# SYSTRAN/faster-whisper

Measured on AMD Instinct MI355X. Metric: audio-sec/sec (RTF) large-v3 fp16 beam=5 batch=16, higher is better.
Workload: dtype f16

## Files before the change

faster_whisper_amd/_lib.py:

```python
import ctypes as C
import os

import numpy as np

_HERE = os.path.dirname(os.path.abspath(__file__))
LIB_PATH = os.environ.get("FWAMD_LIB") or os.path.join(_HERE, "libfwamd.so")

FW_OK = 0
FW_EINVAL = -1
FW_ENODEV = -2
FW_ENOMEM = -3
FW_ERUNTIME = -4
FW_ENOSPC = -5

COMPUTE_FLOAT16 = 0
COMPUTE_INT8_FLOAT16 = 1
FW_DT_F32 = 0
FW_DT_F16 = 1
FW_MAX_ALIGN_HEADS = 64
FW_MAX_ALTERNATIVES = 8


class FwConfig(C.Structure):
    _fields_ = [
        ("n_mels", C.c_int32), ("n_audio_ctx", C.c_int32), ("d_model", C.c_int32), ("n_heads", C.c_int32),
        ("n_enc_layers", C.c_int32), ("n_dec_layers", C.c_int32), ("n_vocab", C.c_int32),
        ("n_text_ctx", C.c_int32), ("is_multilingual", C.c_int32),
        ("tok_eot", C.c_int32), ("tok_sot", C.c_int32), ("tok_lang_begin", C.c_int32), ("n_langs", C.c_int32),
        ("tok_translate", C.c_int32), ("tok_transcribe", C.c_int32), ("tok_sot_lm", C.c_int32),
        ("tok_sot_prev", C.c_int32), ("tok_no_speech", C.c_int32), ("tok_no_timestamps", C.c_int32),
        ("tok_timestamp_begin", C.c_int32),
        ("n_suppress_begin", C.c_int32), ("suppress_begin", C.c_int32 * 8),
        ("n_align_heads", C.c_int32), ("align_heads", C.c_int32 * (2 * FW_MAX_ALIGN_HEADS)),
    ]


class FwWeight(C.Structure):
    _fields_ = [("name", C.c_char_p), ("data", C.c_void_p), ("dtype", C.c_int32), ("ndim", C.c_int32),
                ("dims", C.c_int64 * 4)]


class FwGenOpts(C.Structure):
    _fields_ = [
        ("beam_size", C.c_int32), ("patience", C.c_float), ("num_hypotheses", C.c_int32),
        ("length_penalty", C.c_float), ("repetition_penalty", C.c_float), ("no_repeat_ngram_size", C.c_int32),
        ("max_length", C.c_int32), ("return_scores", C.c_int32), ("return_no_speech_prob", C.c_int32),
        ("max_initial_timestamp_index", C.c_int32), ("suppress_blank", C.c_int32),
        ("suppress_tokens", C.POINTER(C.c_int32)), ("n_suppress_tokens", C.c_int32),
        ("sampling_topk", C.c_int32), ("sampling_temperature", C.c_float), ("seed", C.c_uint64),
        ("min_new_tokens", C.c_int32),
    ]


class FwVadWeights(C.Structure):
    _fields_ = [
        ("stft_basis", C.c_void_p), ("conv_w", C.c_void_p * 4), ("conv_b", C.c_void_p * 4),
        ("lstm_w", C.c_void_p), ("lstm_r", C.c_void_p), ("lstm_b", C.c_void_p), ("dec_w", C.c_void_p),
        ("dec_b", C.c_float),
    ]


SYMBOLS = [
    "fw_last_error", "fw_abi_version", "fw_device_count",
    "fw_model_create", "fw_model_free", "fw_model_info", "fw_model_blob", "fw_model_create_from_blob_dev",
    "fw_model_set_decode_batch", "fw_model_decode_batch", "fw_model_join_decoder", "fw_model_decode_stats",
    "fw_model_set_merge_wait", "fw_model_set_decode_lanes", "fw_model_run_capacity", "fw_dec_big_min_rows", "fw_dec_big_min_rows_of", "fw_test_knob",
    "fw_test_idle_lead_chunks", "fw_test_run_capacity", "fw_test_dec_linear_plan", "fw_test_self_attn_form",
    "fw_test_gemm_plan",
    "fw_pack_blob_size", "fw_pack_blob_copy", "fw_pack_blob_free",
    "fw_logmel", "fw_logmel_full",
    "fw_encode", "fw_encode_pcm", "fw_encode_pcm_dev", "fw_tensor_shape", "fw_tensor_to_host",
    "fw_tensor_from_host", "fw_tensor_free",
    "fw_generate", "fw_generate_lp", "fw_generate_alt", "fw_detect_language", "fw_align", "fw_score",
    "fw_prof_enable", "fw_prof_reset", "fw_prof_count", "fw_prof_name", "fw_prof_get", "fw_synchronize",
    "fw_dev_alloc", "fw_dev_free", "fw_dev_upload",
    "fw_test_gemm", "fw_test_layernorm", "fw_test_attention", "fw_test_dec_linear", "fw_test_dec_logits", "fw_test_logits_rules",
    "fw_test_dec_self_attn", "fw_test_dec_cross_attn", "fw_test_dec_cross_probs", "fw_test_dec_softmax_pick", "fw_bench_gemm", "fw_bench_dec_linear", "fw_bench_attention",
    "fw_bench_gemm_epi", "fw_bench_dec_linear_epi",
    "fw_test_gemm_ex", "fw_test_cross_kv_frag_index", "fw_test_quant_rows", "fw_test_layernorm_frag",
    "fw_test_dec_beam_update", "fw_test_dec_embed", "fw_test_align_post",
    "fw_test_logits_rules_lp", "fw_test_dec_beam_update_lp",
    "fw_test_logits_rules_alt", "fw_test_dec_beam_update_alt", "fw_test_alt_gather",
    "fw_test_logits_rules_smp_tab", "fw_test_logits_rules_ex", "fw_test_score_rows", "fw_test_graph_captures", "fw_test_blob_check",
    "fw_vad_create", "fw_vad_forward", "fw_vad_free", "fw_vad_forward_dev", "fw_vad_forward_audio_dev",
    "fw_vad_forward_audio_batch_dev",
    "fw_flac_info", "fw_flac_decode",
    "fw_resample_filter", "fw_resample_dev", "fw_bench_resample",
]

_lib = None


class FwError(RuntimeError):
    pass


def load():
    global _lib
    if _lib is not None:
        return _lib
    if not os.path.exists(LIB_PATH):
        raise FwError(
            f"{LIB_PATH} not found: build it with `python -c 'import __graft_entry__ as g; g.build()'` "
            "(hipcc --offload-arch=gfx950). faster_whisper_amd has no CPU fallback.")
    lib = C.CDLL(LIB_PATH)
    vp, i32, i64, f32p = C.c_void_p, C.c_int32, C.c_int64, C.POINTER(C.c_float)
    i32p, i64p = C.POINTER(C.c_int32), C.POINTER(C.c_int64)
    lib.fw_last_error.restype = C.c_char_p
    lib.fw_abi_version.restype = i32
    lib.fw_device_count.restype = i32
    lib.fw_model_create.argtypes = [C.POINTER(FwConfig), C.POINTER(FwWeight), i32, i32, i32, i32, i32, C.POINTER(vp)]
    lib.fw_model_free.argtypes = [vp]
    lib.fw_model_free.restype = None
    lib.fw_model_info.argtypes = [vp, C.POINTER(FwConfig), i32p, i32p, i32p, i32p]
    lib.fw_model_blob.argtypes = [vp, C.POINTER(vp), i64p]
    lib.fw_model_create_from_blob_dev.argtypes = [C.POINTER(FwConfig), vp, i64, i32, i32, i32, i32, C.POINTER(vp)]
    lib.fw_model_set_decode_batch.argtypes = [vp, i32]
    lib.fw_model_decode_batch.argtypes = [vp]
    lib.fw_model_decode_batch.restype = i32
    lib.fw_model_run_capacity.argtypes = [vp]
    lib.fw_model_run_capacity.restype = i32
    lib.fw_dec_big_min_rows.restype = i32
    if hasattr(lib, "fw_dec_big_min_rows_of"):
        lib.fw_dec_big_min_rows_of.restype = i32
        lib.fw_dec_big_min_rows_of.argtypes = [i32, i32]
    if hasattr(lib, "fw_flac_info"):
        lib.fw_flac_info.argtypes = [vp, i64, i32p, i32p, i32p, i64p]
        lib.fw_flac_decode.argtypes = [vp, i64, vp, i64, i64p, i32p]
    if hasattr(lib, "fw_test_knob"):
        lib.fw_test_knob.argtypes = [i32, i32]
    if hasattr(lib, "fw_test_idle_lead_chunks"):
        lib.fw_test_idle_lead_chunks.argtypes = [i64, i32, i32, i64, i32]
        lib.fw_test_idle_lead_chunks.restype = i64
    if hasattr(lib, "fw_test_run_capacity"):
        lib.fw_test_run_capacity.argtypes = [i32, i32, i32, i64, i32, i32, i32, i32, i32, i64p, i64p, i64p]
        lib.fw_test_run_capacity.restype = i32
    if hasattr(lib, "fw_test_dec_linear_plan"):
        lib.fw_test_dec_linear_plan.argtypes = [i32, i32, i32, i32, i32, i32, i32, i32p]
        lib.fw_test_self_attn_form.argtypes = [i32] * 8
        lib.fw_test_self_attn_form.restype = i32
    if hasattr(lib, "fw_test_gemm_plan"):
        lib.fw_test_gemm_plan.argtypes = [i32, i32, i32, i32, i64, i64, i64, i64, i64, i32, i32, i32, i32, i32, i32p]
    lib.fw_model_join_decoder.argtypes = [vp, vp]
    lib.fw_model_set_merge_wait.argtypes = [vp, i32, i32]
    lib.fw_model_set_decode_lanes.argtypes = [vp, i32]
    lib.fw_model_decode_stats.argtypes = [vp, i64p, i64p, i64p, i32p]
    lib.fw_pack_blob_size.argtypes = [C.POINTER(FwConfig), C.POINTER(FwWeight), i32, i32, i64p, C.POINTER(vp)]
    lib.fw_pack_blob_copy.argtypes = [vp, vp, i64]
    lib.fw_pack_blob_free.argtypes = [vp]
    lib.fw_pack_blob_free.restype = None
    lib.fw_logmel.argtypes = [vp, vp, i64p, i32, vp, i32p]
    lib.fw_logmel_full.argtypes = [vp, vp, i64, vp, i64]
    lib.fw_encode.argtypes = [vp, vp, i32, C.POINTER(vp)]
    lib.fw_encode_pcm.argtypes = [vp, vp, i64p, i32, C.POINTER(vp)]
    lib.fw_encode_pcm_dev.argtypes = [vp, vp, i64p, i32, C.POINTER(vp)]
    lib.fw_tensor_shape.argtypes = [vp, i32p, i32p, i32p]
    lib.fw_tensor_to_host.argtypes = [vp, vp, vp]
    lib.fw_tensor_from_host.argtypes = [vp, vp, i32, C.POINTER(vp)]
    lib.fw_tensor_free.argtypes = [vp]
    lib.fw_tensor_free.restype = None
    lib.fw_generate.argtypes = [vp, vp, i32p, i32p, i32, C.POINTER(FwGenOpts), i32p, i32p, f32p, f32p]
    if hasattr(lib, "fw_generate_lp"):
        lib.fw_generate_lp.argtypes = [vp, vp, i32p, i32p, i32, C.POINTER(FwGenOpts), i32p, i32p, f32p, f32p, f32p, f32p]
    if hasattr(lib, "fw_generate_alt"):
        f32 = C.c_float
        lib.fw_generate_alt.argtypes = [vp, vp, i32p, i32p, i32, C.POINTER(FwGenOpts), i32, i32p, i32p, f32p, f32p, f32p,
                                        f32p, i32p, f32p, i32p, f32p]
        lib.fw_test_logits_rules_alt.argtypes = [vp, vp, i32, vp, i32, vp, C.POINTER(FwGenOpts), i32, vp, vp, vp, vp, vp,
                                                 vp, vp, i32, vp, vp]
        lib.fw_test_dec_beam_update_alt.argtypes = [vp, i32, i32, i32, i32, i32, i32, i32, i32, f32, i32, vp, vp, vp, vp,
                                                    vp, vp, vp, i32, f32, vp, vp, vp, vp, vp, vp, vp, vp, vp, vp, vp, vp,
                                                    vp, vp, vp]
        lib.fw_test_alt_gather.argtypes = [vp, vp, vp, i32, i32, i32, i32, i32, vp, i32, vp, vp, vp, vp, i32, vp, vp]
    lib.fw_detect_language.argtypes = [vp, vp, i32, i32p, f32p]
    lib.fw_align.argtypes = [vp, vp, i32p, i32, i32p, i32p, i32p, i32, i32, i32, i32p, i32p, f32p]
    lib.fw_prof_enable.argtypes = [vp, i32]
    lib.fw_prof_enable.restype = None
    lib.fw_prof_reset.argtypes = [vp]
    lib.fw_prof_reset.restype = None
    lib.fw_prof_count.restype = i32
    lib.fw_prof_name.argtypes = [i32]
    lib.fw_prof_name.restype = C.c_char_p
    lib.fw_prof_get.argtypes = [vp, i32, C.POINTER(C.c_double), i64p, C.POINTER(C.c_double), C.POINTER(C.c_double)]
    lib.fw_synchronize.argtypes = [vp]
    lib.fw_dev_alloc.argtypes = [vp, i64, C.POINTER(vp)]
    lib.fw_dev_free.argtypes = [vp, vp]
    lib.fw_dev_upload.argtypes = [vp, vp, vp, i64]
    lib.fw_test_gemm.argtypes = [vp, vp, vp, vp, vp, i32, i32, i32, i32, i32, vp]
    lib.fw_test_dec_linear.argtypes = [vp, vp, vp, vp, vp, vp, vp, i32, i32, i32, i32, i32, vp, vp]
    lib.fw_test_dec_logits.argtypes = [vp, vp, i32, vp]
    lib.fw_test_logits_rules.argtypes = [vp, vp, i32, vp, i32, vp, C.POINTER(FwGenOpts), i32, vp, vp]
    if hasattr(lib, "fw_test_dec_self_attn"):
        lib.fw_test_dec_self_attn.argtypes = [vp, vp, vp, vp, vp, i32, i32, i32, i32, i32, i32, i32, i32, i32, i32, i32, vp]
        lib.fw_test_dec_cross_attn.argtypes = [vp, vp, vp, vp, i32, i32, i32, i32, i32, i32, vp, vp, i32, C.c_float, vp]
        lib.fw_test_dec_cross_probs.argtypes = [vp, vp, vp, i32, i32, i32, vp, i32, i32, i32, i32, vp]
# ... 78 lines not shown
```

faster_whisper_amd/csrc/gemm.hip:

```cpp
#include "common.h"
#include "kernels.h"
#include <atomic>
#include <type_traits>

#define GB_M 256
#define GB_N 256
#define GB_UNIT_BYTES (128 * 128)
#define GB_SLOT_BYTES (4 * GB_UNIT_BYTES)
#define GB_LDS_BYTES (8 * 64 * 272)

typedef int intx16 __attribute__((ext_vector_type(16)));

#ifndef GB_TL
#define GB_TL(slot)
#endif

#define GB_BARRIER()                      \
  do {                                    \
    asm volatile("" ::: "memory");         \
    __builtin_amdgcn_s_barrier();         \
    asm volatile("" ::: "memory");         \
  } while (0)

template <bool TRANS, bool I8, bool LAYERED = false>
// ... 406 lines not shown
            if (p.act == 1) v = gelu_erf(v);
            o[e] = (half_t)v;
          }
          half_t* dst = Cb + (size_t)n * p.ldc + m;
          if (m + 3 < p.M) {
            *reinterpret_cast<half4_t*>(dst) = o;
          } else {
#pragma unroll
            for (int e = 0; e < 4; ++e)
              if (m + e < p.M) dst[e] = o[e];
          }
        }
      }
  }
}

namespace fwk {

std::atomic<int> g_gemm_order{1};
std::atomic<int> g_gemm_vt_stage{1};

GemmPlan gemm_plan(const GemmParams& pin, int batch, bool trans) {
  GemmPlan pl{pin, -1, 0};
  GemmParams& p = pl.p;
  const bool i8 = p.a_scale != nullptr, layered = p.n_layers > 1;
  const int es = i8 ? 1 : 2;
  if (p.K <= 0 || (p.K * es) % 128 != 0) return pl;
  if (((p.lda * es) % 16) || ((p.ldw * es) % 16) || ((p.a_bstride * es) % 16)) return pl;
  if (!trans && ((p.N % 4) || (p.ldc % 4) || (p.c_bstride % 4))) return pl;
  if (i8 && !p.w_scale) return pl;
  if (layered && (i8 || p.res)) return pl;
  p.nMt = (p.M + GB_M - 1) / GB_M;
  p.nNt_layer = (p.N + GB_N - 1) / GB_N;
  p.nNt = p.nNt_layer * (layered ? p.n_layers : 1);
  p.n_mp = p.nMt * batch;
  p.blk_m = p.blk_n = 0;
  p.vt_stage = (trans && !i8 && p.head_rows == 0 && g_gemm_vt_stage.load(std::memory_order_relaxed) == 1 && p.ldc % 8 == 0 &&
                p.c_bstride % 8 == 0) ? 1 : 0;
  if (g_gemm_order.load(std::memory_order_relaxed) == 1 && p.nNt > 1 && p.n_mp > 1) {
    int bn = 1, best = 1 << 30;
    for (int c = 1; c <= p.nNt && c <= 16; ++c) {
      if (p.nNt % c) continue;
      const int cost = c + (32 + c - 1) / c;
      if (cost <= best) { best = cost; bn = c; }
    }
    p.blk_n = bn;
    p.blk_m = 32 / bn > 1 ? 32 / bn : 1;
  }
  pl.kernel = layered ? 4 + trans : 2 * i8 + trans;
  pl.grid = p.nMt * p.nNt * batch;
  return pl;
}

int launch_gemm(hipStream_t st, const GemmParams& pin, int batch, bool trans) {
  const GemmPlan pl = gemm_plan(pin, batch, trans);
  if (pl.kernel < 0) return -1;
  static void (*const kernels[6])(GemmParams) = {
      gemm_f16_kernel<false, false>, gemm_f16_kernel<true, false>,       gemm_f16_kernel<false, true>,
      gemm_f16_kernel<true, true>,   gemm_f16_kernel<false, false, true>, gemm_f16_kernel<true, false, true>};
  const int lds = GB_LDS_BYTES;
  static std::atomic<unsigned long long> attr_done{0};
  int dev = 0;
  (void)hipGetDevice(&dev);
  if (!((attr_done.load(std::memory_order_acquire) >> (dev & 63)) & 1ull)) {
    for (auto* k : kernels)
      (void)hipFuncSetAttribute(reinterpret_cast<const void*>(k), hipFuncAttributeMaxDynamicSharedMemorySize, lds);
    attr_done.fetch_or(1ull << (dev & 63), std::memory_order_release);
  }
  hipLaunchKernelGGL(kernels[pl.kernel], dim3(pl.grid), dim3(512), lds, st, pl.p);
  return 0;
}

}
```

faster_whisper_amd/csrc/hooks.hip:

```cpp
#include "engine.h"

#include <math.h>
#include <string.h>

#include <algorithm>

#include "dec_kernels.h"
#include "kernels.h"

using namespace fw;
using fwd::FIN_CAP;
using fwd::GenDev;

namespace {

struct HookBufs : DevBufs {
  template <typename T>
  int upload(T** dst, const T* src, size_t n) {
    int rc = alloc(dst, n);
    if (rc) return rc;
    FW_HIP(hipMemcpy(*dst, src, n * sizeof(T), hipMemcpyHostToDevice));
    return FW_OK;
  }
  int upload_f16(half_t** dst, const float* src, size_t n) {
// ... 182 lines not shown
        (rc = db.upload_f16(&d_x, x, (size_t)R * K)) || (bias && (rc = db.upload_f16(&d_bias, bias, N))) ||
        (rc = db.alloc(&d_xq, (size_t)R16 * K)) || (rc = db.alloc(&d_xs, (size_t)R16)) || (rc = db.zero(d_xq, (size_t)R16 * K, st)))
      return rc;
    fwk::launch_quant_rows(st, d_x, K, nullptr, nullptr, d_xq, d_xs, R, K, 1);
    if (fwd::launch_dec_gemm_frag_i8(st, d_xq, d_xs, d_wq, d_ws, d_bias, d_res, N, d_out, N, R, N, K, act) != 0) {
      set_error("int8 decoder linear: unsupported shape R=%d N=%d K=%d", R, N, K);
      return FW_ERUNTIME;
    }
    if ((rc = download_f16(st, out, d_out, (size_t)R * N))) return rc;
    memcpy(out_from_frag, out, (size_t)R * N * sizeof(float));
    return FW_OK;
  }
  std::vector<uint16_t> wf((size_t)N * K), xf((size_t)R16 * K, 0);
  std::vector<float> s1(N, 0.f), cf(N, 0.f);
  for (int n = 0; n < N; ++n) {
    double a1 = 0.0, ac = 0.0;
    for (int k = 0; k < K; ++k) {
      const float wv = h(W[(size_t)n * K + k]);
      const uint16_t wg = ln_g ? f32_to_f16_bits(wv * h(ln_g[k])) : f32_to_f16_bits(wv);
      wf[frag_pos(n, k, K, 32)] = wg;
      a1 += (double)f16_bits_to_f32(wg);
      if (ln_g) ac += (double)wv * (double)h(ln_b[k]);
    }
    if (bias) ac += (double)h(bias[n]);
    s1[n] = (float)a1;
    cf[n] = (float)ac;
  }
  for (int r = 0; r < R; ++r)
    for (int k = 0; k < K; ++k) xf[frag_pos(r, k, K, 32)] = f32_to_f16_bits(x[(size_t)r * K + k]);
  uint16_t *d_wf, *d_xf;
  half_t* d_of;
  float *d_s1 = nullptr, *d_cf = nullptr;
  if ((rc = db.upload(&d_wf, wf.data(), wf.size())) || (rc = db.upload(&d_xf, xf.data(), xf.size())) ||
      (rc = db.alloc(&d_of, (size_t)R16 * N)) || (rc = db.zero(d_of, (size_t)R16 * N * 2, st)))
    return rc;
  if (ln_g) {
    if ((rc = db.upload(&d_s1, s1.data(), (size_t)N)) || (rc = db.upload(&d_cf, cf.data(), (size_t)N))) return rc;
  } else if (bias) {
    if ((rc = db.upload_f16(&d_bias, bias, N))) return rc;
  }
  const fwd::DecLin lin{(const half_t*)d_xf, (const half_t*)d_wf, d_bias, d_s1, d_cf, d_res, N, d_out, N, d_of, R, N, K, act};
  if (fwd::launch_dec_linear(st, lin, form) != 0) {
    set_error("decoder linear: unsupported shape R=%d N=%d K=%d (form %d)", R, N, K, form);
    return FW_ERUNTIME;
  }
  if ((rc = download_f16(st, out, d_out, (size_t)R * N))) return rc;
  return download_f16_frag(st, out_from_frag, d_of, R, N);
}

int32_t fw_dec_big_min_rows(void) { return fwd::dec_big_min_rows(); }
int32_t fw_dec_big_min_rows_of(int32_t role, int32_t compute_type) { return fwd::dec_big_min_rows_of(role, compute_type); }

int32_t fw_test_knob(int32_t id, int32_t value) {
  FW_CHECK_ARG(id == 1 || id == 2 || id == 4 || id == 5 || id == 6 || id == 7, "unknown knob %d", id);
  if (id == 6) { set_cross_kv_layered(value); return FW_OK; }
  if (id == 7) { fwd::set_cross_attn_regs(value); return FW_OK; }
  if (id == 1) fwk::g_gemm_order.store(value);
  else if (id == 5) fwk::g_gemm_vt_stage.store(value);
  else if (id == 2) fwd::set_self_attn_form(value);
  else set_pos_blocks(value);
  return FW_OK;
}

int64_t fw_test_idle_lead_chunks(int64_t queued, int32_t n_queued, int32_t encoding, int64_t want, int32_t max_batch) {
  return idle_lead_chunks(queued, n_queued, encoding, want, max_batch);
}

int32_t fw_test_run_capacity(int32_t lane_chunks, int32_t max_batch, int32_t max_beam, int64_t self_cap, int32_t B,
                             int32_t sampling, int32_t beam_size, int32_t num_hypotheses, int32_t ctx,
                             int64_t* rows_per_chunk, int64_t* want, int64_t* run_cap) {
  const RunCapacity cap(lane_chunks, max_batch, max_beam, self_cap, B, sampling != 0, beam_size, num_hypotheses, ctx);
  *rows_per_chunk = cap.rows_per_chunk;
  *want = cap.want;
  *run_cap = cap.run_cap;
  return cap.rows_fit && cap.cache_fits ? 1 : 0;
}

int32_t fw_test_dec_linear_plan(int32_t R, int32_t N, int32_t K, int32_t ldo, int32_t ldr, int32_t compute_type,
                                int32_t form, int32_t out[6]) {
  const fwd::DecLinPlan p = fwd::dec_linear_plan(R, N, K, ldo, ldr, compute_type, form);
  const int32_t f[6] = {p.family, p.cfg, p.row_tiles, p.col_tiles, p.chunk, p.waves};
  memcpy(out, f, sizeof(f));
  return FW_OK;
}

int32_t fw_test_gemm_plan(int32_t M, int32_t N, int32_t K, int32_t batch, int64_t lda, int64_t ldw, int64_t a_bstride,
                          int64_t ldc, int64_t c_bstride, int32_t trans, int32_t int8, int32_t head_rows, int32_t n_layers,
                          int32_t has_res, int32_t out[9]) {
  static const float some_scale = 1.f;
  static const half_t some_res = 0;
  fwk::GemmParams p{};
  p.lda = lda; p.a_bstride = a_bstride; p.ldw = ldw; p.ldc = ldc; p.c_bstride = c_bstride;
  p.M = M; p.N = N; p.K = K;
  p.head_rows = head_rows; p.n_layers = n_layers;
  p.a_scale = int8 ? &some_scale : nullptr;
  p.w_scale = int8 == 1 ? &some_scale : nullptr;
  p.res = has_res ? &some_res : nullptr;
  const fwk::GemmPlan pl = fwk::gemm_plan(p, batch, trans != 0);
  const int32_t f[9] = {pl.kernel, pl.p.nMt, pl.p.nNt, pl.p.nNt_layer, pl.p.n_mp, pl.p.blk_n, pl.p.blk_m, pl.p.vt_stage, pl.grid};
  memcpy(out, f, sizeof(f));
  return FW_OK;
}

int32_t fw_test_self_attn_form(int32_t n_ctx, int32_t cache_ctx, int32_t d, int32_t R_total, int32_t kmul, int32_t H,
                               int32_t chunks, int32_t knob) {
  return fwd::self_attn_form(n_ctx, cache_ctx, d, R_total, kmul, H, chunks, knob);
}

int32_t fw_test_blob_check(const void* blob_host, int64_t bytes) {
  FW_CHECK_ARG(blob_host && bytes >= (int64_t)sizeof(BlobHeader), "weight blob too small");
  BlobHeader h;
  memcpy(&h, blob_host, sizeof(h));
  if (int rc = check_blob_header(h, bytes)) return rc;
  std::vector<BlobEntry> entries(h.n_tensors);
  memcpy(entries.data(), reinterpret_cast<const char*>(blob_host) + sizeof(h), entries.size() * sizeof(BlobEntry));
  Weights unused;
  bool has_plain;
  return bind_weights(h, entries.data(), const_cast<void*>(blob_host), unused, &has_plain);
}

int32_t fw_test_dec_logits(fw_model* fm, const float* x, int32_t R, float* out) {
  FW_CHECK_ARG(fm && x && out && R >= 1, "bad argument");
  Model* m = &fm->impl;
  std::lock_guard<std::mutex> lk(m->mu);
  FW_HIP(hipSetDevice(m->device));
  hipStream_t st = m->stream;
  const int d = m->cfg.d_model, V = m->cfg.n_vocab, R16 = (R + 15) / 16 * 16;
  const bool i8 = m->compute_type == FW_COMPUTE_INT8_FLOAT16;
  std::vector<half_t> xh((size_t)R16 * d, (half_t)0.f);
  for (int r = 0; r < R; ++r)
    for (int k = 0; k < d; ++k) xh[i8 ? (size_t)r * d + k : frag_pos(r, k, d, 32)] = (half_t)x[(size_t)r * d + k];
  HookBufs db;
  half_t* d_x;
  float* d_out;
  int rc, lr;
  if ((rc = db.upload(&d_x, xh.data(), xh.size())) || (rc = db.alloc(&d_out, (size_t)R * V))) return rc;
  if (i8) {
    int8_t* d_xq;
    float* d_xs;
    if ((rc = db.alloc(&d_xq, (size_t)R16 * d)) || (rc = db.alloc(&d_xs, (size_t)R16)) || (rc = db.zero(d_xq, (size_t)R16 * d, st)))
      return rc;
    fwk::launch_quant_rows(st, d_x, d, m->dec_ln.g, m->dec_ln.b, d_xq, d_xs, R, d, 1);
    lr = fwd::launch_dec_logits(st, true, d_xq, d_xs, m->logits.wq, m->logits.wscale, nullptr, nullptr, d_out, V, R, V, d);
  } else {
    lr = fwd::launch_dec_logits(st, false, d_x, nullptr, m->logits.w, nullptr, m->logits.s1, m->logits.cf, d_out, V, R, V,
                                d);
  }
  FW_HIP(hipStreamSynchronize(st));
  if (lr != 0) {
    set_error("logits projection test failed: unsupported shape");
    return FW_ERUNTIME;
  }
  return download(out, d_out, (size_t)R * V);
}

int32_t fw_bench_dec_linear(fw_model* fm, int32_t R, int32_t N, int32_t K, int32_t lnf, int32_t variant, int32_t iters,
// ... 109 lines not shown
  *ms_out = ms / (float)iters;
  return FW_OK;
}

int32_t fw_bench_dec_linear_epi(fw_model* fm, int32_t R, int32_t N, int32_t K, int32_t lnf, int32_t variant, int32_t act,
                                int32_t res, int32_t outs, int32_t iters, float* us_out) {
  FW_CHECK_ARG(fm && us_out && R > 0 && N > 0 && K > 0 && iters > 0, "bad argument");
  FW_CHECK_ARG((outs & 3) != 0 && (!res || (outs & 1)), "needs an output; the residual is the row-major output in place");
  FW_CHECK_ARG(variant == 0 || variant == 5 || (variant >= 10 && variant <= 12), "unknown variant %d", variant);
  Model* m = &fm->impl;
  std::lock_guard<std::mutex> lk(m->mu);
  FW_HIP(hipSetDevice(m->device));
  hipStream_t st = m->stream;
  const size_t wn = (size_t)N * K;
  const int copies = (int)std::max<size_t>(2, ((size_t)640 << 20) / (wn * 2));
  const size_t rp = ((size_t)R + 15) / 16 * 16, on = rp * N;
  const int ocopies = (int)std::max<size_t>(2, ((size_t)640 << 20) / (on * 2));
  HookBufs db;
  half_t *dW, *dX, *dO, *dF, *dB;
  float *dS, *dC;
  std::vector<uint16_t> stage;
  int rc;
  if ((rc = db.alloc(&dW, wn * copies)) || (rc = db.alloc(&dX, rp * K)) || (rc = db.alloc(&dO, on * ocopies)) ||
      (rc = db.alloc(&dF, on)) || (rc = db.alloc(&dB, (size_t)N)) || (rc = db.alloc(&dS, (size_t)N)) || (rc = db.alloc(&dC, (size_t)N)) ||
      (rc = fill_lcg(dW, wn, stage, 2463534242u, 1e-3f)) || (rc = fill_lcg(dX, rp * K, stage, 2463534242u, 1e-3f)) ||
      (rc = db.zero(dO, on * ocopies * 2, st)) || (rc = db.zero(dB, (size_t)N * 2, st)) || (rc = db.zero(dS, (size_t)N * 4, st)) ||
      (rc = db.zero(dC, (size_t)N * 4, st)))
    return rc;
  for (int c = 1; c < copies; ++c) FW_HIP(hipMemcpy(dW + (size_t)c * wn, dW, wn * 2, hipMemcpyDeviceToDevice));
  float ms = 0.f;
  rc = time_launches(st, 4, iters, [&](int i) {
    const half_t* w = dW + (size_t)(i % copies) * wn;
    half_t* o = dO + (size_t)(i % ocopies) * on;
    half_t* op = (outs & 1) ? o : nullptr;
    half_t* of = (outs & 2) ? dF : nullptr;
    const half_t* r = res ? o : nullptr;
    const half_t* b = lnf ? nullptr : dB;
    const float *s1 = lnf ? dS : nullptr, *cf = lnf ? dC : nullptr;
    return fwd::launch_dec_linear(st, fwd::DecLin{dX, w, b, s1, cf, r, N, op, N, of, R, N, K, act}, variant);
  }, &ms);
  if (rc == LAUNCH_REFUSED) { set_error("fw_bench_dec_linear_epi: unsupported shape / variant"); return FW_EINVAL; }
  if (rc) return rc;
  *us_out = ms * 1000.f / (float)iters;
  return FW_OK;
}

int32_t fw_test_layernorm(fw_model* fm, const float* x, const float* g, const float* b, int32_t rows, int32_t d,
                          float* out) {
  return test_layernorm_impl(fm, x, g, b, rows, d, 0, out);
}
int32_t fw_test_layernorm_frag(fw_model* fm, const float* x, const float* g, const float* b, int32_t rows, int32_t d,
                               int32_t frag, float* out) {
  return test_layernorm_impl(fm, x, g, b, rows, d, frag, out);
}

int32_t fw_test_quant_rows(fw_model* fm, const float* x, int32_t rows, int32_t d, int64_t ldx, const float* ln_g,
                           const float* ln_b, int32_t frag, int8_t* xq, float* scale) {
  FW_CHECK_ARG(fm && x && xq && scale && rows >= 1 && rows <= (1 << 20), "bad argument");
  FW_CHECK_ARG((ln_g == nullptr) == (ln_b == nullptr), "ln_g and ln_b go together");
  FW_CHECK_ARG(d >= 64 && d % 64 == 0 && d <= (ln_g ? 1536 : 5120), "d %% 64 == 0, d <= 1536 with LayerNorm, <= 5120 without");
  FW_CHECK_ARG(ldx >= d && ldx % 8 == 0 && ldx <= (1 << 20), "ldx >= d, ldx %% 8 == 0");
  Model* m = &fm->impl;
  std::lock_guard<std::mutex> lk(m->mu);
  FW_HIP(hipSetDevice(m->device));
  const int R16 = (rows + 15) / 16 * 16;
  std::vector<int8_t> hq((size_t)R16 * d);
  HookBufs db;
  half_t *dx, *dg = nullptr, *dlb = nullptr;
  int8_t* dq;
  float* ds;
  int rc;
  if ((rc = db.upload_f16(&dx, x, (size_t)(rows - 1) * ldx + d)) || (ln_g && (rc = db.upload_f16(&dg, ln_g, d))) ||
      (ln_b && (rc = db.upload_f16(&dlb, ln_b, d))) || (rc = db.alloc(&dq, hq.size())) || (rc = db.alloc(&ds, (size_t)R16)) ||
      (rc = db.zero(dq, hq.size(), m->stream)))
    return rc;
  fwk::launch_quant_rows(m->stream, dx, ldx, dg, dlb, dq, ds, rows, d, frag ? 1 : 0);
  FW_HIP(hipStreamSynchronize(m->stream));
  if ((rc = download(hq.data(), dq, hq.size())) || (rc = download(scale, ds, (size_t)rows))) return rc;
  for (int r = 0; r < rows; ++r)
    for (int k = 0; k < d; ++k) xq[(size_t)r * d + k] = hq[frag ? frag_pos(r, k, d, 64) : (size_t)r * d + k];
  return FW_OK;
}

int32_t fw_test_cross_kv_frag_index(int32_t vt, int32_t kvp, int32_t N, int64_t* idx) {
  FW_CHECK_ARG(idx && kvp >= 32 && kvp % 32 == 0 && N >= 64 && N % 64 == 0, "need kvp %% 32 == 0, N %% 64 == 0");
  for (int mm = 0; mm < kvp; ++mm)
    for (int n = 0; n < N; ++n) idx[(size_t)mm * N + n] = (int64_t)cross_kv_frag_pos(vt != 0, kvp, mm, n);
  return FW_OK;
}

int32_t fw_test_gemm_ex(fw_model* fm, const float* A, int64_t a_elems, int64_t lda, int64_t a_bstride, const float* W,
                        const float* bias, const float* res, int64_t r_elems, int64_t ldr, int64_t r_bstride, float* C,
                        int64_t c_elems, int64_t c_off, int64_t ldc, int64_t c_bstride, int64_t c_lstride, int32_t M,
                        int32_t N, int32_t K, int32_t batch, int32_t n_layers, int32_t act, int32_t trans,
                        int32_t head_rows, int32_t use_int8, const float* ln_g, const float* ln_b) {
  FW_CHECK_ARG(fm && A && W && C, "null argument");
  const int64_t dim_max = 1 << 20, cnt_max = 1 << 12, str_max = (int64_t)1 << 40;
  FW_CHECK_ARG(M >= 1 && N >= 1 && K >= 1 && M <= dim_max && N <= dim_max && K <= dim_max, "bad M / N / K");
  FW_CHECK_ARG(batch >= 1 && n_layers >= 1 && batch <= cnt_max && n_layers <= cnt_max, "bad batch / n_layers");
  for (int64_t v : {a_elems, lda, a_bstride, r_elems, ldr, r_bstride, c_elems, c_off, ldc, c_bstride, c_lstride})
    FW_CHECK_ARG(v >= 0 && v <= str_max, "negative or oversized count / stride");
  FW_CHECK_ARG(act == 0 || act == 1, "act is 0 or 1");
  FW_CHECK_ARG((ln_g == nullptr) == (ln_b == nullptr) && (!ln_g || use_int8), "ln_g / ln_b: both, and only with use_int8");
  const bool rowmajor = !trans && head_rows == 0;
  FW_CHECK_ARG(!res || (rowmajor && n_layers == 1), "a residual needs the row-major single-layer form");
  FW_CHECK_ARG(n_layers == 1 || (!use_int8 && act == 0), "the layered launch is fp16 without activation");
// ... 718 lines not shown
```

faster_whisper_amd/csrc/kernels.h:

```cpp
#pragma once
#include <atomic>
#include "common.h"

namespace fwk {

size_t logmel_lds_bytes();
void launch_logmel(hipStream_t st, const float* pcm_dev, const int64_t* offsets_dev, int B, int max_frames_total,
                   const float* consts, const float* filtT, int mel_pad, int n_mels, float* raw,
                   int64_t raw_bstride, int raw_stride, int* chunk_max, int drop_last, int out_frames,
                   float* out_f32, half_t* out_cl, int c_pad, int* n_frames_out);
void launch_features_to_cl(hipStream_t st, const float* feats_dev, int B, int n_mels, int frames, half_t* out_cl,
                           int c_pad);

struct GemmParams {
  const half_t* A; int64_t lda; int64_t a_bstride;
  const half_t* W; int64_t ldw;
  const half_t* bias;
  const half_t* res; int64_t ldr; int64_t r_bstride;
  half_t* C; int64_t ldc; int64_t c_bstride;
  int M, N, K;
  int act;
  int head_rows;
  const float* a_scale; int64_t as_bstride; const float* w_scale;
  int nMt, nNt;
  int n_mp, blk_m, blk_n;
  int vt_stage;
  int n_layers; int64_t w_lstride, bias_lstride, c_lstride;
  int nNt_layer;
};
struct GemmPlan {
  GemmParams p;
  int kernel;
  int grid;
};
GemmPlan gemm_plan(const GemmParams& p, int batch, bool trans);
int launch_gemm(hipStream_t st, const GemmParams& p, int batch, bool trans);
extern std::atomic<int> g_gemm_order;
extern std::atomic<int> g_gemm_vt_stage;

void launch_layernorm(hipStream_t st, const half_t* x, const half_t* g, const half_t* b, half_t* y, int rows, int d,
                      int frag = 0);
void launch_quant_rows(hipStream_t st, const half_t* x, int64_t ldx, const half_t* g, const half_t* b, int8_t* xq,
                       float* scale, int rows, int d, int frag = 0);
void launch_f32_to_f16(hipStream_t st, const float* x, half_t* y, int64_t n);
void launch_f16_to_f32(hipStream_t st, const half_t* x, float* y, int64_t n);

struct AttnEnc {
  const half_t *q, *k; int64_t ld, qk_bstride;
  const half_t* vt; int64_t ldvt, vt_bstride;
  half_t* out; int64_t ldo, o_bstride;
  int B, H, T;
  int order = 0;
};
void launch_attn_enc(hipStream_t st, const AttnEnc& a);

}
```

faster_whisper_amd/csrc/rowops.hip:

```cpp
#include "common.h"
#include "kernels.h"

#define LN_MAXC 3
#define QR_MAXC 10

template <int MAXC>
static __device__ __forceinline__ float load_row(const half_t* xr, int nc, int lane, float (&v)[MAXC][8]) {
  float s = 0.f;
#pragma unroll
  for (int i = 0; i < MAXC; ++i) {
    const int c = i * 64 + lane;
    if (c < nc) {
      const half8_t h = *reinterpret_cast<const half8_t*>(xr + (size_t)c * 8);
#pragma unroll
      for (int e = 0; e < 8; ++e) { v[i][e] = (float)h[e]; s += v[i][e]; }
    } else {
#pragma unroll
      for (int e = 0; e < 8; ++e) v[i][e] = 0.f;
    }
  }
  return s;
}

template <int MAXC>
static __device__ __forceinline__ float normalise_row(float (&v)[MAXC][8], int nc, int lane, int d, float sum,
                                                      const half_t* g, const half_t* b) {
  const float mean = wave_sum(sum) / (float)d;
  float q = 0.f;
#pragma unroll
  for (int i = 0; i < MAXC; ++i)
    if (i * 64 + lane < nc) {
#pragma unroll
      for (int e = 0; e < 8; ++e) { const float a = v[i][e] - mean; q += a * a; }
    }
  const float rstd = rsqrtf(wave_sum(q) / (float)d + 1e-5f);
  float amax = 0.f;
#pragma unroll
  for (int i = 0; i < MAXC; ++i) {
    const int c = i * 64 + lane;
    if (c < nc) {
      const half8_t gg = *reinterpret_cast<const half8_t*>(g + (size_t)c * 8);
      const half8_t bb = *reinterpret_cast<const half8_t*>(b + (size_t)c * 8);
#pragma unroll
      for (int e = 0; e < 8; ++e) {
        v[i][e] = (float)(half_t)((v[i][e] - mean) * rstd * (float)gg[e] + (float)bb[e]);
        amax = fmaxf(amax, fabsf(v[i][e]));
      }
    }
  }
  return amax;
}

__global__ __launch_bounds__(256) void layernorm_kernel(const half_t* __restrict__ x, const half_t* __restrict__ g,
                                                        const half_t* __restrict__ b, half_t* __restrict__ y,
                                                        int rows, int d, int frag) {
  const int lane = threadIdx.x & 63;
  const int row = blockIdx.x * 4 + (threadIdx.x >> 6);
  if (row >= rows) return;
  const int nc = d >> 3;
  float v[LN_MAXC][8];
  const float s = load_row<LN_MAXC>(x + (size_t)row * d, nc, lane, v);
  (void)normalise_row<LN_MAXC>(v, nc, lane, d, s, g, b);
  half_t* yr = y + (size_t)row * d;
#pragma unroll
  for (int i = 0; i < LN_MAXC; ++i) {
    const int c = i * 64 + lane;
    if (c < nc) {
      half8_t o;
#pragma unroll
      for (int e = 0; e < 8; ++e) o[e] = (half_t)v[i][e];
      if (frag)
        *reinterpret_cast<half8_t*>(y + ((size_t)((row >> 4) * (d >> 5) + (c >> 2)) * 64 + (c & 3) * 16 + (row & 15)) * 8) = o;
      else
        *reinterpret_cast<half8_t*>(yr + (size_t)c * 8) = o;
    }
  }
}

template <int MAXC, bool LN>
static __device__ __forceinline__ void quant_row(const half_t* xr, const half_t* g, const half_t* b, int8_t* xq,
                                                 float* scale, int row, int d, int frag, int lane) {
  const int nc = d >> 3;
  float v[MAXC][8];
  const float s = load_row<MAXC>(xr, nc, lane, v);
  float amax = 0.f;
  if (LN) {
    amax = normalise_row<MAXC>(v, nc, lane, d, s, g, b);
  } else {
#pragma unroll
    for (int i = 0; i < MAXC; ++i)
#pragma unroll
      for (int e = 0; e < 8; ++e) amax = fmaxf(amax, fabsf(v[i][e]));
  }
  amax = wave_max(amax);
  const float inv = amax > 0.f ? 127.0f / amax : 0.f;
  if (lane == 0) scale[row] = amax > 0.f ? amax / 127.0f : 1.0f;
#pragma unroll
  for (int i = 0; i < MAXC; ++i) {
    const int c = i * 64 + lane;
    if (c < nc) {
      union { signed char q[8]; intx2 w; } o;
#pragma unroll
      for (int e = 0; e < 8; ++e) o.q[e] = (signed char)__float2int_rn(v[i][e] * inv);
      const int k = c * 8;
      const size_t off = frag ? ((size_t)((row >> 4) * (d >> 6) + (k >> 6)) * 64 + ((k >> 4) & 3) * 16 + (row & 15)) * 16 + (k & 15)
                              : (size_t)row * d + k;
      *reinterpret_cast<intx2*>(xq + off) = o.w;
    }
  }
}

__global__ __launch_bounds__(256) void quant_rows_kernel(const half_t* __restrict__ x, int64_t ldx,
                                                         const half_t* __restrict__ g, const half_t* __restrict__ b,
                                                         int8_t* __restrict__ xq, float* __restrict__ scale, int rows,
                                                         int d, int frag) {
  const int lane = threadIdx.x & 63;
  const int row = blockIdx.x * 4 + (threadIdx.x >> 6);
  if (row >= rows) return;
  const half_t* xr = x + (size_t)row * ldx;
  if (g) quant_row<LN_MAXC, true>(xr, g, b, xq, scale, row, d, frag, lane);
  else if (d <= 8 * 64 * LN_MAXC) quant_row<LN_MAXC, false>(xr, g, b, xq, scale, row, d, frag, lane);
  else quant_row<QR_MAXC, false>(xr, g, b, xq, scale, row, d, frag, lane);
}

__global__ void f32_to_f16_kernel(const float* __restrict__ x, half_t* __restrict__ y, int64_t n) {
  int64_t i = (int64_t)blockIdx.x * blockDim.x + threadIdx.x;
  const int64_t stride = (int64_t)gridDim.x * blockDim.x;
  for (; i < n; i += stride) y[i] = (half_t)x[i];
}
__global__ void f16_to_f32_kernel(const half_t* __restrict__ x, float* __restrict__ y, int64_t n) {
  int64_t i = (int64_t)blockIdx.x * blockDim.x + threadIdx.x;
  const int64_t stride = (int64_t)gridDim.x * blockDim.x;
  for (; i < n; i += stride) y[i] = (float)x[i];
}

namespace fwk {
void launch_layernorm(hipStream_t st, const half_t* x, const half_t* g, const half_t* b, half_t* y, int rows, int d,
                      int frag) {
  layernorm_kernel<<<(rows + 3) / 4, 256, 0, st>>>(x, g, b, y, rows, d, frag);
}
// ... 16 lines not shown
```

Before: 3190.

## Flatten dense batched GEMMs into one tall GEMM and prefetch layernorm loads

When batch slices of A, C and residual are contiguous, the batched GEMM is replanned as a single GEMM with M*batch rows, so tiles span batch boundaries and fewer M tiles are wasted on padding. This is on by default and can be turned off with a new knob. The row kernels now issue the x, gamma and beta loads up front, before the reductions, to overlap memory latency, and layernorm switches to a different wave-sum variant. New test and bench hooks for both changes are added as well.

```diff
diff --git a/faster_whisper_amd/_lib.py b/faster_whisper_amd/_lib.py
--- a/faster_whisper_amd/_lib.py
+++ b/faster_whisper_amd/_lib.py
@@ -66,7 +66,7 @@
     "fw_model_set_decode_batch", "fw_model_decode_batch", "fw_model_join_decoder", "fw_model_decode_stats",
     "fw_model_set_merge_wait", "fw_model_set_decode_lanes", "fw_model_run_capacity", "fw_dec_big_min_rows", "fw_dec_big_min_rows_of", "fw_test_knob",
     "fw_test_idle_lead_chunks", "fw_test_run_capacity", "fw_test_dec_linear_plan", "fw_test_self_attn_form",
-    "fw_test_gemm_plan",
+    "fw_test_gemm_plan", "fw_test_gemm_launch_plan", "fw_test_layernorm_ex", "fw_bench_layernorm",
     "fw_pack_blob_size", "fw_pack_blob_copy", "fw_pack_blob_free",
     "fw_logmel", "fw_logmel_full",
     "fw_encode", "fw_encode_pcm", "fw_encode_pcm_dev", "fw_tensor_shape", "fw_tensor_to_host",
@@ -141,6 +141,11 @@
         lib.fw_test_self_attn_form.restype = i32
     if hasattr(lib, "fw_test_gemm_plan"):
         lib.fw_test_gemm_plan.argtypes = [i32, i32, i32, i32, i64, i64, i64, i64, i64, i32, i32, i32, i32, i32, i32p]
+    if hasattr(lib, "fw_test_gemm_launch_plan"):
+        lib.fw_test_gemm_launch_plan.argtypes = [i32, i32, i32, i32, i64, i64, i64, i64, i64, i32, i64, i64, i32, i64, i32,
+                                                 i32, i32, i32p]
+        lib.fw_test_layernorm_ex.argtypes = [vp, vp, vp, vp, i32, i32, i32, vp, i64]
+        lib.fw_bench_layernorm.argtypes = [vp, i32, i32, i32, i32, f32p]
     lib.fw_model_join_decoder.argtypes = [vp, vp]
     lib.fw_model_set_merge_wait.argtypes = [vp, i32, i32]
     lib.fw_model_set_decode_lanes.argtypes = [vp, i32]
diff --git a/faster_whisper_amd/csrc/gemm.hip b/faster_whisper_amd/csrc/gemm.hip
--- a/faster_whisper_amd/csrc/gemm.hip
+++ b/faster_whisper_amd/csrc/gemm.hip
@@ -482,8 +482,29 @@
   return pl;
 }
 
+std::atomic<int> g_gemm_dense_rows{1};
+
+bool gemm_dense_rows(const GemmParams& p, int batch, bool trans) {
+  if (g_gemm_dense_rows.load(std::memory_order_relaxed) != 1) return false;
+  if (batch <= 1 || trans || p.head_rows != 0 || p.n_layers > 1 || p.M <= 0) return false;
+  const int64_t M = p.M, rows = M * batch;
+  if (p.a_bstride != M * p.lda || p.c_bstride != M * p.ldc) return false;
+  if (p.res && p.r_bstride != M * p.ldr) return false;
+  if (p.a_scale && p.as_bstride != M) return false;
+  const int64_t es = p.a_scale ? 1 : 2;
+  if (rows > INT32_MAX || p.lda <= 0 || rows - 1 > (((int64_t)1 << 32) - 1 - p.K * es) / (p.lda * es)) return false;
+  return true;
+}
+
+GemmPlan gemm_launch_plan(const GemmParams& pin, int batch, bool trans) {
+  if (!gemm_dense_rows(pin, batch, trans)) return gemm_plan(pin, batch, trans);
+  GemmParams p = pin;
+  p.M = pin.M * batch;
+  return gemm_plan(p, 1, trans);
+}
+
 int launch_gemm(hipStream_t st, const GemmParams& pin, int batch, bool trans) {
-  const GemmPlan pl = gemm_plan(pin, batch, trans);
+  const GemmPlan pl = gemm_launch_plan(pin, batch, trans);
   if (pl.kernel < 0) return -1;
   static void (*const kernels[6])(GemmParams) = {
       gemm_f16_kernel<false, false>, gemm_f16_kernel<true, false>,       gemm_f16_kernel<false, true>,
diff --git a/faster_whisper_amd/csrc/hooks.hip b/faster_whisper_amd/csrc/hooks.hip
--- a/faster_whisper_amd/csrc/hooks.hip
+++ b/faster_whisper_amd/csrc/hooks.hip
@@ -258,8 +258,9 @@
 int32_t fw_dec_big_min_rows_of(int32_t role, int32_t compute_type) { return fwd::dec_big_min_rows_of(role, compute_type); }
 
 int32_t fw_test_knob(int32_t id, int32_t value) {
-  FW_CHECK_ARG(id == 1 || id == 2 || id == 4 || id == 5 || id == 6 || id == 7, "unknown knob %d", id);
+  FW_CHECK_ARG(id == 1 || id == 2 || id == 4 || id == 5 || id == 6 || id == 7 || id == 8, "unknown knob %d", id);
   if (id == 6) { set_cross_kv_layered(value); return FW_OK; }
+  if (id == 8) { fwk::g_gemm_dense_rows.store(value); return FW_OK; }
   if (id == 7) { fwd::set_cross_attn_regs(value); return FW_OK; }
   if (id == 1) fwk::g_gemm_order.store(value);
   else if (id == 5) fwk::g_gemm_vt_stage.store(value);
@@ -308,6 +309,27 @@
   return FW_OK;
 }
 
+int32_t fw_test_gemm_launch_plan(int32_t M, int32_t N, int32_t K, int32_t batch, int64_t lda, int64_t ldw, int64_t a_bstride,
+                                 int64_t ldc, int64_t c_bstride, int32_t has_res, int64_t ldr, int64_t r_bstride,
+                                 int32_t int8, int64_t as_bstride, int32_t trans, int32_t head_rows, int32_t n_layers,
+                                 int32_t out[11]) {
+  static const float some_scale = 1.f;
+  static const half_t some_res = 0;
+  fwk::GemmParams p{};
+  p.lda = lda; p.a_bstride = a_bstride; p.ldw = ldw; p.ldc = ldc; p.c_bstride = c_bstride;
+  p.M = M; p.N = N; p.K = K;
+  p.head_rows = head_rows; p.n_layers = n_layers;
+  p.a_scale = int8 ? &some_scale : nullptr; p.as_bstride = as_bstride;
+  p.w_scale = int8 ? &some_scale : nullptr;
+  p.res = has_res ? &some_res : nullptr; p.ldr = ldr; p.r_bstride = r_bstride;
+  const fwk::GemmPlan pl = fwk::gemm_launch_plan(p, batch, trans != 0);
+  const int32_t chunks = pl.p.nMt > 0 ? pl.p.n_mp / pl.p.nMt : 0;
+  const int32_t f[11] = {pl.kernel, pl.p.nMt, pl.p.nNt, pl.p.nNt_layer, pl.p.n_mp, pl.p.blk_n, pl.p.blk_m, pl.p.vt_stage, pl.grid,
+                         chunks,    pl.p.M};
+  memcpy(out, f, sizeof(f));
+  return FW_OK;
+}
+
 int32_t fw_test_self_attn_form(int32_t n_ctx, int32_t cache_ctx, int32_t d, int32_t R_total, int32_t kmul, int32_t H,
                                int32_t chunks, int32_t knob) {
   return fwd::self_attn_form(n_ctx, cache_ctx, d, R_total, kmul, H, chunks, knob);
@@ -523,6 +545,53 @@
 int32_t fw_test_layernorm_frag(fw_model* fm, const float* x, const float* g, const float* b, int32_t rows, int32_t d,
                                int32_t frag, float* out) {
   return test_layernorm_impl(fm, x, g, b, rows, d, frag, out);
+}
+
+int32_t fw_test_layernorm_ex(fw_model* fm, const float* x, const float* g, const float* b, int32_t rows, int32_t d,
+                             int32_t frag, float* y, int64_t y_elems) {
+  FW_CHECK_ARG(fm && x && g && b && y && rows >= 1 && rows <= (1 << 20), "bad argument");
+  FW_CHECK_ARG(d >= 8 && d % 8 == 0 && d <= 1536 && (!frag || d % 32 == 0), "d %% 8 == 0 (fragment-major: %% 32), d <= 1536");
+  const int64_t need = (int64_t)(frag ? (rows + 15) / 16 * 16 : rows) * d;
+  FW_CHECK_ARG(y_elems >= need, "the launch writes up to y[%lld], y_elems = %lld", (long long)need - 1, (long long)y_elems);
+  Model* m = &fm->impl;
+  std::lock_guard<std::mutex> lk(m->mu);
+  FW_HIP(hipSetDevice(m->device));
+  HookBufs db;
+  half_t *dx, *dg, *dlb, *dy;
+  int rc;
+  if ((rc = db.upload_f16(&dx, x, (size_t)rows * d)) || (rc = db.upload_f16(&dg, g, d)) || (rc = db.upload_f16(&dlb, b, d)) ||
+      (rc = db.upload_f16(&dy, y, (size_t)y_elems)))
+    return rc;
+  fwk::launch_layernorm(m->stream, dx, dg, dlb, dy, rows, d, frag ? 1 : 0);
+  return download_f16(m->stream, y, dy, (size_t)y_elems);
+}
+
+int32_t fw_bench_layernorm(fw_model* fm, int32_t rows, int32_t d, int32_t frag, int32_t iters, float* us_out) {
+  FW_CHECK_ARG(fm && us_out && rows >= 1 && rows <= (1 << 20) && iters > 0, "bad argument");
+  FW_CHECK_ARG(d >= 8 && d % 8 == 0 && d <= 1536 && (!frag || d % 32 == 0), "d %% 8 == 0 (fragment-major: %% 32), d <= 1536");
+  Model* m = &fm->impl;
+  std::lock_guard<std::mutex> lk(m->mu);
+  FW_HIP(hipSetDevice(m->device));
+  hipStream_t st = m->stream;
+  const size_t n = (size_t)(rows + 15) / 16 * 16 * d;
+  const int copies = (int)std::max<size_t>(2, ((size_t)640 << 20) / (n * 2) + 1);
+  HookBufs db;
+  half_t *dX, *dY, *dG, *dB;
+  std::vector<uint16_t> stage;
+  int rc;
+  if ((rc = db.alloc(&dX, n * copies)) || (rc = db.alloc(&dY, n * copies)) || (rc = db.alloc(&dG, (size_t)d)) ||
+      (rc = db.alloc(&dB, (size_t)d)) || (rc = fill_lcg(dX, n, stage, 2463534242u, 1e-3f)) ||
+      (rc = fill_lcg(dG, (size_t)d, stage, 777u, 1e-3f)) || (rc = fill_lcg(dB, (size_t)d, stage, 4242u, 1e-3f)))
+    return rc;
+  for (int c = 1; c < copies; ++c) FW_HIP(hipMemcpy(dX + (size_t)c * n, dX, n * 2, hipMemcpyDeviceToDevice));
+  float ms = 0.f;
+  rc = time_launches(st, 4, iters, [&](int i) {
+    fwk::launch_layernorm(st, dX + (size_t)(i % copies) * n, dG, dB, dY + (size_t)(i % copies) * n, rows, d, frag ? 1 : 0);
+    return 0;
+  }, &ms);
+  if (rc) return rc;
+  *us_out = ms * 1000.f / (float)iters;
+  return FW_OK;
 }
 
 int32_t fw_test_quant_rows(fw_model* fm, const float* x, int32_t rows, int32_t d, int64_t ldx, const float* ln_g,
diff --git a/faster_whisper_amd/csrc/kernels.h b/faster_whisper_amd/csrc/kernels.h
--- a/faster_whisper_amd/csrc/kernels.h
+++ b/faster_whisper_amd/csrc/kernels.h
@@ -34,8 +34,11 @@
   int grid;
 };
 GemmPlan gemm_plan(const GemmParams& p, int batch, bool trans);
+bool gemm_dense_rows(const GemmParams& p, int batch, bool trans);
+GemmPlan gemm_launch_plan(const GemmParams& p, int batch, bool trans);
 int launch_gemm(hipStream_t st, const GemmParams& p, int batch, bool trans);
 extern std::atomic<int> g_gemm_order;
+extern std::atomic<int> g_gemm_dense_rows;
 extern std::atomic<int> g_gemm_vt_stage;
 
 void launch_layernorm(hipStream_t st, const half_t* x, const half_t* g, const half_t* b, half_t* y, int rows, int d,
diff --git a/faster_whisper_amd/csrc/rowops.hip b/faster_whisper_amd/csrc/rowops.hip
--- a/faster_whisper_amd/csrc/rowops.hip
+++ b/faster_whisper_amd/csrc/rowops.hip
@@ -5,15 +5,27 @@
 #define QR_MAXC 10
 
 template <int MAXC>
-static __device__ __forceinline__ float load_row(const half_t* xr, int nc, int lane, float (&v)[MAXC][8]) {
-  float s = 0.f;
+static __device__ __forceinline__ void fetch_row(const half_t* xr, int nc, int lane, half8_t (&h)[MAXC]) {
 #pragma unroll
   for (int i = 0; i < MAXC; ++i) {
     const int c = i * 64 + lane;
     if (c < nc) {
-      const half8_t h = *reinterpret_cast<const half8_t*>(xr + (size_t)c * 8);
+      h[i] = *reinterpret_cast<const half8_t*>(xr + (size_t)c * 8);
+    } else {
 #pragma unroll
-      for (int e = 0; e < 8; ++e) { v[i][e] = (float)h[e]; s += v[i][e]; }
+      for (int e = 0; e < 8; ++e) h[i][e] = (half_t)0.f;
+    }
+  }
+}
+
+template <int MAXC>
+static __device__ __forceinline__ float sum_row(const half8_t (&h)[MAXC], int nc, int lane, float (&v)[MAXC][8]) {
+  float s = 0.f;
+#pragma unroll
+  for (int i = 0; i < MAXC; ++i) {
+    if (i * 64 + lane < nc) {
+#pragma unroll
+      for (int e = 0; e < 8; ++e) { v[i][e] = (float)h[i][e]; s += v[i][e]; }
     } else {
 #pragma unroll
       for (int e = 0; e < 8; ++e) v[i][e] = 0.f;
@@ -22,10 +34,10 @@
   return s;
 }
 
-template <int MAXC>
-static __device__ __forceinline__ float normalise_row(float (&v)[MAXC][8], int nc, int lane, int d, float sum,
-                                                      const half_t* g, const half_t* b) {
-  const float mean = wave_sum(sum) / (float)d;
+template <int MAXC, bool VSUM = false>
+static __device__ __forceinline__ void row_stats(const float (&v)[MAXC][8], int nc, int lane, int d, float sum, float& mean,
+                                                 float& rstd) {
+  mean = (VSUM ? wave_sum_v(sum) : wave_sum(sum)) / (float)d;
   float q = 0.f;
 #pragma unroll
   for (int i = 0; i < MAXC; ++i)
@@ -33,17 +45,19 @@
 #pragma unroll
       for (int e = 0; e < 8; ++e) { const float a = v[i][e] - mean; q += a * a; }
     }
-  const float rstd = rsqrtf(wave_sum(q) / (float)d + 1e-5f);
+  rstd = rsqrtf((VSUM ? wave_sum_v(q) : wave_sum(q)) / (float)d + 1e-5f);
+}
+
+template <int MAXC>
+static __device__ __forceinline__ float scale_row(float (&v)[MAXC][8], int nc, int lane, float mean, float rstd,
+                                                  const half8_t (&gg)[MAXC], const half8_t (&bb)[MAXC]) {
   float amax = 0.f;
 #pragma unroll
   for (int i = 0; i < MAXC; ++i) {
-    const int c = i * 64 + lane;
-    if (c < nc) {
-      const half8_t gg = *reinterpret_cast<const half8_t*>(g + (size_t)c * 8);
-      const half8_t bb = *reinterpret_cast<const half8_t*>(b + (size_t)c * 8);
+    if (i * 64 + lane < nc) {
 #pragma unroll
       for (int e = 0; e < 8; ++e) {
-        v[i][e] = (float)(half_t)((v[i][e] - mean) * rstd * (float)gg[e] + (float)bb[e]);
+        v[i][e] = (float)(half_t)((v[i][e] - mean) * rstd * (float)gg[i][e] + (float)bb[i][e]);
         amax = fmaxf(amax, fabsf(v[i][e]));
       }
     }
@@ -58,9 +72,14 @@
   const int row = blockIdx.x * 4 + (threadIdx.x >> 6);
   if (row >= rows) return;
   const int nc = d >> 3;
-  float v[LN_MAXC][8];
-  const float s = load_row<LN_MAXC>(x + (size_t)row * d, nc, lane, v);
-  (void)normalise_row<LN_MAXC>(v, nc, lane, d, s, g, b);
+  half8_t h[LN_MAXC], gg[LN_MAXC], bb[LN_MAXC];
+  fetch_row<LN_MAXC>(x + (size_t)row * d, nc, lane, h);
+  fetch_row<LN_MAXC>(g, nc, lane, gg);
+  fetch_row<LN_MAXC>(b, nc, lane, bb);
+  float v[LN_MAXC][8], mean, rstd;
+  const float s = sum_row<LN_MAXC>(h, nc, lane, v);
+  row_stats<LN_MAXC, true>(v, nc, lane, d, s, mean, rstd);
+  (void)scale_row<LN_MAXC>(v, nc, lane, mean, rstd, gg, bb);
   half_t* yr = y + (size_t)row * d;
 #pragma unroll
   for (int i = 0; i < LN_MAXC; ++i) {
@@ -81,11 +100,19 @@
 static __device__ __forceinline__ void quant_row(const half_t* xr, const half_t* g, const half_t* b, int8_t* xq,
                                                  float* scale, int row, int d, int frag, int lane) {
   const int nc = d >> 3;
+  half8_t gg[MAXC], bb[MAXC], h[MAXC];
+  if constexpr (LN) {
+    fetch_row<MAXC>(g, nc, lane, gg);
+    fetch_row<MAXC>(b, nc, lane, bb);
+  }
+  fetch_row<MAXC>(xr, nc, lane, h);
   float v[MAXC][8];
-  const float s = load_row<MAXC>(xr, nc, lane, v);
+  const float s = sum_row<MAXC>(h, nc, lane, v);
   float amax = 0.f;
-  if (LN) {
-    amax = normalise_row<MAXC>(v, nc, lane, d, s, g, b);
+  if constexpr (LN) {
+    float mean, rstd;
+    row_stats<MAXC>(v, nc, lane, d, s, mean, rstd);
+    amax = scale_row<MAXC>(v, nc, lane, mean, rstd, gg, bb);
   } else {
 #pragma unroll
     for (int i = 0; i < MAXC; ++i)
diff --git a/profiles/layernorm_bench.py b/profiles/layernorm_bench.py
--- /dev/null
+++ b/profiles/layernorm_bench.py
@@ -0,0 +1,32 @@
+import argparse
+import ctypes as C
+import json
+import os
+import sys
+
+sys.path.insert(0, os.path.dirname(os.path.dirname(os.path.abspath(__file__))))
+
+
+def main():
+    ap = argparse.ArgumentParser()
+    ap.add_argument("--rounds", type=int, default=3)
+    ap.add_argument("--iters", type=int, default=200)
+    ap.add_argument("--rows", type=int, default=24000)
+    ap.add_argument("--d", type=int, default=1280)
+    a = ap.parse_args()
+    from faster_whisper_amd import Whisper, _lib, get_config, synthetic_weights
+    cfg = get_config("micro")
+    model = Whisper("synthetic:micro", device="cuda", files={"config": cfg, "weights": synthetic_weights(cfg, 3)},
+                    compute_type="float16", max_batch_size=1, max_beam_size=1)
+    lib = _lib.load()
+    h = model._replicas[0].handle
+    nbytes = 4.0 * a.rows * a.d
+    for rnd in range(a.rounds):
+        us = C.c_float()
+        _lib.check(lib.fw_bench_layernorm(h, a.rows, a.d, 0, a.iters, C.byref(us)))
+        print(json.dumps({"round": rnd, "lib": _lib.LIB_PATH, "us": round(us.value, 2),
+                          "TB/s": round(nbytes / us.value / 1e6, 3)}), flush=True)
+
+
+if __name__ == "__main__":
+    main()
```

Result: no change. 3200 (median of 2 runs) (+0.3%).
